# GATB/MindTheGap

Hardware: AMD Instinct MI355X
Metric: breakpoints filled/sec (higher is better)
Workload: dtype u64; 1 GPU; synthetic human-scale: 3 Gbp i.i.d. donor as 600000 x 5 kb sequences, 100000 insertion sites (50-1000 nt) per batch, k=31, max-nodes 100; sites_per_batch=100000, sites_per_rank_and_step=100000, distinct_batches_per_rank=4, site_set=400000, donor_sequences=600000, erroneous_fragments=0, k=31, max_nodes=100, max_length=10000, nb_solid_kmers=3108581096, nb_unitigs=600024, index_bytes=60154587216, unitig_store_bytes=3945966160, batches_in_flight=6, input=prepared batches, resident in HBM, output=C-ABI records + ASCII sequences in page-locked host memory

## Files before the change

### mindthegap_amd/csrc/mtg_gpu_fill.hip

```cpp
#include "mtg_gpu_common.h"

namespace mtgi {

enum { TRAVERSAL_SETS = mtg_index::NWS };
__constant__ Index c_ix[TRAVERSAL_SETS];
__constant__ FillCfg c_cfg[TRAVERSAL_SETS];

#ifndef MTG_STAGE_A_WAVES
#define MTG_STAGE_A_WAVES 2
#endif
#ifndef MTG_WALK_WAVES
#define MTG_WALK_WAVES 2
#endif
enum { PARK_LISTS = 19 };
struct ParkCtl {
    uint32_t count[PARK_LISTS];
    uint32_t n_branching;
    uint32_t pad_[3];
#ifdef MTG_BUBBLE_TIMING
    uint32_t hist_lane[32], hist_wave[32], hist_walk_lane[32], hist_walk_wave[32];
#endif
};
#ifdef MTG_BUBBLE_TIMING
__device__ __forceinline__ void timing_note(uint32_t* hl, uint32_t* hw, uint64_t t0)
// ... 950 lines not shown
            const uint32_t general_hint = ws.post_general == ~0u ? m : (uint32_t)std::min<uint64_t>(m, 4ull * ws.post_general + 1024ull);
            hipLaunchKernelGGL(k_post, dim3(general_hint), dim3(64), 0, stream, idx->dev, cfg, d_raw.as<uint8_t>(), d_head.as<uint8_t>(), d_out.as<GapOut>(), ids, d_tle, d_tbad, d_toff, d_tcnt, d_mis, d_fok,
                               in.want_all_contigs ? 1u : 0u, d_rec.as<SlotRec>(), m, park, (const uint32_t*)d_pi_head, (const uint32_t*)d_pi_next, pi_mask, d_rw, d_roff, d_tie_p);
            hipLaunchKernelGGL(k_post_lean, dim3((m + 64 / POST_LEAN_G - 1) / (64 / POST_LEAN_G)), dim3(64), 0, stream, idx->dev, cfg, d_raw.as<uint8_t>(), d_head.as<uint8_t>(), d_out.as<GapOut>(), in.want_all_contigs ? 1u : 0u, d_rec.as<SlotRec>(), m);
            const ScanBegin sbegin{{0, 0, arena_used[0], arena_used[1]}};
            hipLaunchKernelGGL(k_scan1, dim3(nblocks), dim3(SCAN_SL), 0, stream, d_rec.as<SlotRec>(), m, d_blocks.as<ScanBlock>());
            hipLaunchKernelGGL(k_scan2, dim3(1), dim3(256), 0, stream, d_blocks.as<ScanBlock>(), nblocks, sbegin, d_tot.as<PartTot>(), h_tot, park);
            HIP_TRY(hipGetLastError());
            EmitDev D;
            EmitHost H;
            const double share = std::min(1.0, std::max(0.0, tune::f(tune::T_PACKED_SEQ_SHARE, 0.0)));
            const uint32_t pack_q = (uint32_t)std::lround(share * 65536.0);
            bool packed = want_records && combo && identity && arena_used[0] == 0 && pack_q != 0;
            uint64_t shadow_halves = 0;
            if (packed) {
                shadow_halves = 2 * ((((uint64_t)sink.seq_cap * pack_q) >> 16) / 32 + 3);
                HIP_TRY(d_shadow.alloc(shadow_halves * 4));
            }
            auto emit = [&]() -> int {
                D.seq = sink.seq_dev ? sink.seq_dev : p_seq(); D.ext = d_ext.as<char>();
                D.seq_cap = sink.seq_cap; D.ext_cap = sink.ext_cap;
                D.res = p_res(); D.fil = p_fil();
                D.dense_words = d_dw.as<uint64_t>(); D.dense_meta = d_dm.as<uint32_t>();
                D.dense_cap_words = ws.cap[d_dw.slot] / 8; D.dense_cap_contigs = ws.cap[d_dm.slot] / 20;
                const bool want_wire = sink.wire_dev != nullptr && identity && tier == 0;
                D.wire = want_wire ? (uint8_t*)sink.wire_dev : nullptr; D.wire_cap = sink.wire_cap; D.wire_tag = sink.wire_tag;
                D.tot = d_tot.as<PartTot>(); D.wire_gaps = m;
                D.shadow = packed ? d_shadow.as<uint32_t>() : nullptr; D.shadow_cap = shadow_halves; D.pack_q = pack_q;
                if (packed) HIP_TRY(hipMemsetAsync(d_shadow.p, 0, shadow_halves * 4, stream));
                if (want_wire) HIP_TRY(hipMemsetAsync(sink.wire_dev, 0, sizeof(mtg_wire_header), stream));
                H.seq = sink.seq; H.ext = sink.ext; H.fil = sink.fil;
                if (!want_wire)
                    hipLaunchKernelGGL(k_emit_lean, dim3((m + 64 / EMIT_LEAN_G - 1) / (64 / EMIT_LEAN_G)), dim3(64), 0, stream, idx->dev.us, cfg, d_raw.as<uint8_t>(), d_head.as<uint8_t>(), d_rec.as<SlotRec>(), d_blocks.as<ScanBlock>(),
                                       ids, d_flags, k, D, H, m);
                hipLaunchKernelGGL(k_emit, dim3(want_wire ? m : general_hint), dim3(64), 0, stream, idx->dev.us, cfg, d_raw.as<uint8_t>(), d_head.as<uint8_t>(), d_rec.as<SlotRec>(), d_blocks.as<ScanBlock>(), ids, d_flags, k, D, H,
                                   d_rlist.as<uint32_t>(), d_glist.as<uint32_t>(), m, park, want_wire ? 0u : 1u);
                if (want_wire) hipLaunchKernelGGL(k_wire_sum, dim3(256 * 4), dim3(256), 0, stream, (uint8_t*)sink.wire_dev, sink.wire_cap);
                HIP_TRY(hipGetLastError());
                return MTG_OK;
            };
            HIP_TRY(mark(eve));
            if (int erc = emit()) return erc;
            HIP_TRY(hipEventRecord(ev2, stream));
            tick("host prep+launch");
            if (while_busy && !busy_done) { busy_done = true; (*while_busy)(); tick("host work during kernels"); }
            HIP_TRY(hipEventSynchronize(ev2));
            traversal_lock.unlock();
            tick("totals ready");
            t0 = now_ms();
            PartTot tot = *h_tot;
            const uint64_t need_w = tot.end[0] * 8 + 64, need_m = tot.end[1] * 20 + 64;
            bool again = false;
            if (want_records && tot.end[2] > sink.seq_cap) {
                const uintptr_t old = (uintptr_t)sink.seq, old_end = old + sink.seq_cap;
                const uintptr_t old_fil = (uintptr_t)sink.fil, old_fil_end = old_fil + n * sizeof(mtg_filled);
                if (!sink.grow_seq || !sink.grow_seq((size_t)tot.end[2], (size_t)tot.begin[2])) { set_error("sequence buffer too small: %llu bytes needed", (unsigned long long)tot.end[2]); return MTG_ERR_ARG; }
                if (launches > 1 && (uintptr_t)sink.seq != old)
                    for (size_t i = 0; i < n; i++) { const uintptr_t q = (uintptr_t)sink.fil[i].seq; if (q >= old && q < old_end) sink.fil[i].seq = sink.seq + (q - old); }
                if (launches > 1 && (uintptr_t)sink.fil != old_fil)
                    for (size_t i = 0; i < n; i++) { const uintptr_t q = (uintptr_t)sink.res[i].filled; if (q >= old_fil && q < old_fil_end) sink.res[i].filled = (const mtg_filled*)((const char*)sink.fil + (q - old_fil)); }
                again = true;
            }
            if (want_records && tot.end[3] > sink.ext_cap) {
                const uintptr_t old = (uintptr_t)sink.ext, old_end = old + sink.ext_cap;
                if (!sink.grow_ext || !sink.grow_ext((size_t)tot.end[3], (size_t)tot.begin[3])) { set_error("extension buffer too small: %llu bytes needed", (unsigned long long)tot.end[3]); return MTG_ERR_NOMEM; }
                if (launches > 1 && (uintptr_t)sink.ext != old)
                    for (size_t i = 0; i < n; i++) { const uintptr_t q = (uintptr_t)sink.res[i].extension; if (q >= old && q < old_end) sink.res[i].extension = sink.ext + (q - old); }
                again = true;
            }
            if (need_w > ws.cap[d_dw.slot] || need_m > ws.cap[d_dm.slot]) again = true;
            if (again) {
                HIP_TRY(hipStreamSynchronize(stream));
                if (combo) HIP_TRY(d_combo.grow_keeping(sink.combo_off_seq + std::max<size_t>(sink.seq_cap, 64) + SEQ_SLACK, sink.combo_off_seq + (size_t)tot.begin[2]));
                else if (!sink.seq_dev) HIP_TRY(d_seq.grow_keeping(std::max<size_t>(sink.seq_cap, 64) + SEQ_SLACK, (size_t)tot.begin[2]));
                HIP_TRY(d_ext.alloc(std::max<size_t>(sink.ext_cap, 64)));
                HIP_TRY(d_dw.alloc(need_w));
                HIP_TRY(d_dm.alloc(need_m));
                hipLaunchKernelGGL(k_scan1, dim3(nblocks), dim3(SCAN_SL), 0, stream, d_rec.as<SlotRec>(), m, d_blocks.as<ScanBlock>());
                hipLaunchKernelGGL(k_scan2, dim3(1), dim3(256), 0, stream, d_blocks.as<ScanBlock>(), nblocks, sbegin, d_tot.as<PartTot>(), (PartTot*)nullptr, park);
                packed = false;
                if (int erc = emit()) return erc;
            }
            CopyTurn copy_turn(idx->device);
            std::vector<mtg_gap_result> tmp_res;
            std::vector<mtg_filled> tmp_fil;
            const bool one_copy = combo && identity && tot.begin[2] == 0;
            const uint64_t pack_x = packed ? packed_split(tot.end[2], pack_q) : 0, pack_words = packed ? (tot.end[2] - pack_x + 31) / 32 : 0;
            uint64_t* h_shadow = nullptr;
            if (packed) {
                h_shadow = (uint64_t*)staging_host(&ws, Workspace::NHOST - 3, pack_words * 8 + 64);
                if (!h_shadow) { set_error("no page-locked memory for the packed sequences of a launch"); return MTG_ERR_NOMEM; }
            }
            if (want_records) {
                if (h_shadow) {
                    HIP_TRY(hipMemcpyAsync(sink.combo, d_combo.p, sink.combo_off_seq, hipMemcpyDeviceToHost, stream));
                    if (pack_words) HIP_TRY(hipMemcpyAsync(h_shadow, d_shadow.p, pack_words * 8, hipMemcpyDeviceToHost, stream));
                    HIP_TRY(hipEventRecord(evp, stream));
                    if (pack_x) HIP_TRY(hipMemcpyAsync(sink.combo + sink.combo_off_seq, (const char*)d_combo.p + sink.combo_off_seq, pack_x, hipMemcpyDeviceToHost, stream));
                } else if (one_copy) HIP_TRY(hipMemcpyAsync(sink.combo, d_combo.p, sink.combo_off_seq + (size_t)tot.end[2], hipMemcpyDeviceToHost, stream));
                else if (identity) {
                    HIP_TRY(hipMemcpyAsync(sink.res, p_res(), (size_t)m * sizeof(mtg_gap_result), hipMemcpyDeviceToHost, stream));
                    HIP_TRY(hipMemcpyAsync(sink.fil, p_fil(), (size_t)m * sizeof(mtg_filled), hipMemcpyDeviceToHost, stream));
                } else {
                    tmp_res.resize(m);
                    tmp_fil.resize(m);
                    HIP_TRY(hipMemcpyAsync(tmp_res.data(), p_res(), (size_t)m * sizeof(mtg_gap_result), hipMemcpyDeviceToHost, stream));
                    HIP_TRY(hipMemcpyAsync(tmp_fil.data(), p_fil(), (size_t)m * sizeof(mtg_filled), hipMemcpyDeviceToHost, stream));
                }
                const WireLayout wl = wire_layout(m, tot.n_filled, tot.end[2], tot.end[3]);
                const bool wired = sink.wire_dev != nullptr && identity && tier == 0 && wl.total <= sink.wire_cap && tot.n_retry == 0 && tot.n_general == 0;
                if (sink.wire_dev && identity && tier == 0) { sink.wire_ok = wired; sink.wire_bytes = wired ? wl.total : 0; }
                const char* seq_src = wired ? (const char*)sink.wire_dev + wl.o_seq : (sink.seq_dev ? sink.seq_dev : p_seq());
                if (!one_copy && !sink.seq_on_device && !sink.seq_stays_in_workspace && tot.end[2] > tot.begin[2]) HIP_TRY(hipMemcpyAsync(sink.seq + tot.begin[2], seq_src + tot.begin[2], tot.end[2] - tot.begin[2], hipMemcpyDeviceToHost, stream));
                if (tot.end[3] > tot.begin[3]) HIP_TRY(hipMemcpyAsync(sink.ext + tot.begin[3], d_ext.as<char>() + tot.begin[3], tot.end[3] - tot.begin[3], hipMemcpyDeviceToHost, stream));
            }
            std::vector<uint32_t> rlist(tot.n_retry), glist(tot.n_general);
            const bool dev_general = tot.n_general > 0 && !host_paths && !in.want_all_contigs && !tune::on(tune::T_HOST_GENERAL) && !tl_host_general;
            GenCtl* h_gctl = nullptr;
            GenDev GD{};
            if (dev_general) {
                const uint64_t ng = tot.n_general;
                HIP_TRY(d_paths.alloc(ng * (size_t)PATHS_WORDS * 4));
                HIP_TRY(d_ggaps.alloc(ng * sizeof(GenGap) + sizeof(GenCtl)));
                GD.cap_sols = 4 * ng + 1024; GD.cap_ascii = ng * 1280 + (1u << 20); GD.cap_tmp = ng * 48 + (1u << 17); GD.cap_bnd = 1u << 22;
                HIP_TRY(d_gsols.alloc(GD.cap_sols * sizeof(GenSol)));
                HIP_TRY(d_gascii.alloc(GD.cap_ascii + 64));
                HIP_TRY(d_gtmp.alloc(GD.cap_tmp * 8));
                HIP_TRY(d_gbnd.alloc(GD.cap_bnd * sizeof(NwCell)));
                GD.ctl = (GenCtl*)d_ggaps.p;
                GD.gaps = (GenGap*)((char*)d_ggaps.p + sizeof(GenCtl));
                GD.sols = d_gsols.as<GenSol>(); GD.ascii = d_gascii.as<char>(); GD.tmp = d_gtmp.as<uint64_t>(); GD.bnd = d_gbnd.as<NwCell>();
                HIP_TRY(hipMemsetAsync(GD.ctl, 0, sizeof(GenCtl), stream));
                hipLaunchKernelGGL(k_paths, dim3((unsigned)ng), dim3(64), 0, stream, cfg, d_raw.as<uint8_t>(), d_head.as<uint8_t>(), d_out.as<GapOut>(), d_glist.as<uint32_t>(), k, d_paths.as<uint32_t>(), (uint32_t)ng);
                hipLaunchKernelGGL(k_general, dim3((unsigned)ng), dim3(64), 0, stream, idx->dev, cfg, d_raw.as<uint8_t>(), d_head.as<uint8_t>(), d_out.as<GapOut>(), d_glist.as<uint32_t>(), ids, d_paths.as<uint32_t>(),
                                   d_tcnt, d_fok, d_src, d_flags, k, GD, (uint32_t)ng);
                HIP_TRY(hipGetLastError());
                h_gctl = (GenCtl*)staging_host(&ws, Workspace::NHOST - 2, sizeof(GenCtl) + ng * sizeof(GenGap) + 64);
                if (!h_gctl) { set_error("no page-locked memory for the multi-contig gaps of a launch"); return MTG_ERR_NOMEM; }
                HIP_TRY(hipMemcpyAsync(h_gctl, d_ggaps.p, sizeof(GenCtl) + ng * sizeof(GenGap), hipMemcpyDeviceToHost, stream));
            }
            HostChunk* hc = nullptr;
            SlotRec* h_rec = nullptr;
            uint64_t* h_w = nullptr;
            uint32_t* h_m = nullptr;
            const uint64_t tw = tot.end[0], tc = tot.end[1];
            if (tot.n_retry) HIP_TRY(hipMemcpyAsync(rlist.data(), d_rlist.p, (size_t)tot.n_retry * 4, hipMemcpyDeviceToHost, stream));
            auto contigs_to_host = [&]() -> int {
                hc->carve(m, tw, tc, h_rec, h_w, h_m);
                HIP_TRY(hipMemcpyAsync(h_rec, d_rec.p, (size_t)m * sizeof(SlotRec), hipMemcpyDeviceToHost, stream));
                if (tw) HIP_TRY(hipMemcpyAsync(h_w, d_dw.p, tw * 8, hipMemcpyDeviceToHost, stream));
                if (tc) HIP_TRY(hipMemcpyAsync(h_m, d_dm.p, tc * 20, hipMemcpyDeviceToHost, stream));
                return MTG_OK;
            };
            if (tot.n_general) {
                special.chunks.emplace_back(new HostChunk());
                hc = special.chunks.back().get();
                HIP_TRY(hipMemcpyAsync(glist.data(), d_glist.p, (size_t)tot.n_general * 4, hipMemcpyDeviceToHost, stream));
                if (!dev_general) { if (int crc = contigs_to_host()) return crc; }
            }
            HIP_TRY(hipEventRecord(ev3, stream));
            if (h_shadow) {
                HIP_TRY(hipEventSynchronize(evp));
                const double tx = now_ms();
                expand_packed_tail(h_shadow, sink.seq, pack_x, tot.end[2], sink.res, sink.fil, n, std::min(8, std::max(1, Pool::cpu_budget() / 2)));
                if (dbg) fprintf(stderr, "  [device_run] %-18s %.3f ms (%llu of %llu arena bytes from %llu words)\n", "packed tail", now_ms() - tx,
                                 (unsigned long long)(tot.end[2] - pack_x), (unsigned long long)tot.end[2], (unsigned long long)pack_words);
            }
            HIP_TRY(hipEventSynchronize(ev3));
            copy_turn.release();
            st.d2h_ms += now_ms() - t0;
            tick("results on the host");
            t0 = now_ms();
            st.index_lines += tot.lines; st.contig_nt += tot.contig_nt; st.store_runs += tot.store_runs; st.run_nt += tot.run_nt; st.post_lines += tot.post_lines;
            st.contig_words += tot.contig_words; st.coverage_kmers += tot.cov_kmers; st.dense_words += tw;
            st.copy_words += tot.copy_words; st.copy_cmds += tot.copy_cmds; st.coverage_direct_kmers += tot.cov_direct; st.n_lean_gaps += tot.n_lean;
            if (tier == 0 && identity) ws.post_general = m - (uint32_t)std::min<uint64_t>(tot.n_lean, m);
            st.copy_words_executed += tot.copy_words_exec; st.copy_cmds_executed += tot.copy_cmds_exec; st.post_scanned_words += tot.scan_words;
            sink.seq_used = tot.end[2];
            sink.ext_used = tot.end[3];
            arena_used[0] = tot.end[2];
            arena_used[1] = tot.end[3];
            sink.n_filled += tot.n_filled;
            if (want_records && !identity)
                for (uint32_t s2 = 0; s2 < m; s2++) { sink.res[host_ids[s2]] = tmp_res[s2]; sink.fil[host_ids[s2]] = tmp_fil[s2]; }
            for (uint32_t s2 : rlist) retry.push_back(host_ids ? host_ids[s2] : s2);
            if (tot.n_retry) sink.in_gap_order = false;
            if (hc && dev_general) {
                const uint64_t ng = tot.n_general;
                const GenCtl ctl = *h_gctl;
                const GenGap* hg = (const GenGap*)(h_gctl + 1);
                hc->gen_gaps.assign(hg, hg + ng);
                uint64_t n_host = 0;
                for (uint64_t i = 0; i < ng; i++) n_host += hg[i].status != GEN_OK;
                const uint64_t ns = std::min<uint64_t>(ctl.n_sols, GD.cap_sols), na = std::min<uint64_t>(ctl.ascii_bytes, GD.cap_ascii);
                hc->gen_sols.resize(ns);
                hc->gen_ascii.resize(na + 1);
                if (ns) HIP_TRY(hipMemcpyAsync(hc->gen_sols.data(), d_gsols.p, ns * sizeof(GenSol), hipMemcpyDeviceToHost, stream));
                if (na) HIP_TRY(hipMemcpyAsync(hc->gen_ascii.data(), d_gascii.p, na, hipMemcpyDeviceToHost, stream));
                if (host_ids) hc->gap_of.assign(host_ids, host_ids + m);
                const uint32_t chunk_id = (uint32_t)special.chunks.size() - 1;
                for (uint32_t i = 0; i < (uint32_t)ng; i++) special.special.push_back(SpecialGap{host_ids ? host_ids[glist[i]] : glist[i], chunk_id, glist[i], i});
                if (n_host) {
                    if (int crc = contigs_to_host()) return crc;
                    hc->path_of.assign(m, -1);
                    if (2 * n_host > ng) {
                        hc->paths.resize(ng * (size_t)PATHS_WORDS);
                        HIP_TRY(hipMemcpyAsync(hc->paths.data(), d_paths.p, ng * (size_t)PATHS_WORDS * 4, hipMemcpyDeviceToHost, stream));
                        for (uint32_t i = 0; i < (uint32_t)ng; i++) if (hg[i].status != GEN_OK) hc->path_of[glist[i]] = (int32_t)i;
                    } else {
                        hc->paths.resize(n_host * (size_t)PATHS_WORDS);
                        uint64_t q = 0;
                        for (uint32_t i = 0; i < (uint32_t)ng; i++)
                            if (hg[i].status != GEN_OK) {
                                HIP_TRY(hipMemcpyAsync(hc->paths.data() + q * PATHS_WORDS, d_paths.as<uint32_t>() + (size_t)i * PATHS_WORDS, (size_t)PATHS_WORDS * 4, hipMemcpyDeviceToHost, stream));
                                hc->path_of[glist[i]] = (int32_t)q++;
                            }
                    }
                }
                HIP_TRY(hipStreamSynchronize(stream));
                if (n_host) h_w[tw] = 0;
                st.n_general_host += n_host;
                st.n_general_device += ng - n_host;
            } else if (hc) {
                h_w[tw] = 0;
                if (host_ids) hc->gap_of.assign(host_ids, host_ids + m);
                const uint32_t chunk_id = (uint32_t)special.chunks.size() - 1;
                std::vector<uint32_t> pslots;
                st.n_general_host += glist.size();
                uint32_t grank = 0;
                for (uint32_t s2 : glist) {
                    special.special.push_back(SpecialGap{host_ids ? host_ids[s2] : s2, chunk_id, s2, grank++});
                    if (!host_paths && !in.want_all_contigs && h_rec[s2].p.fast == 0 && h_rec[s2].p.nb_terminal > 0) pslots.push_back(s2);
                }
                if (!pslots.empty()) {
                    HIP_TRY(d_ids.alloc(std::max<size_t>(chunk, pslots.size()) * 4));
                    HIP_TRY(hipMemcpyAsync(d_ids.p, pslots.data(), pslots.size() * 4, hipMemcpyHostToDevice, stream));
                    HIP_TRY(d_paths.alloc(pslots.size() * (size_t)PATHS_WORDS * 4));
                    hipLaunchKernelGGL(k_paths, dim3((unsigned)pslots.size()), dim3(64), 0, stream, cfg, d_raw.as<uint8_t>(), d_head.as<uint8_t>(), d_out.as<GapOut>(), d_ids.as<uint32_t>(), k,
                                       d_paths.as<uint32_t>(), (uint32_t)pslots.size());
                    HIP_TRY(hipGetLastError());
                    hc->paths.resize(pslots.size() * (size_t)PATHS_WORDS);
                    HIP_TRY(hipMemcpyAsync(hc->paths.data(), d_paths.p, hc->paths.size() * 4, hipMemcpyDeviceToHost, stream));
                    HIP_TRY(hipStreamSynchronize(stream));
                    hc->path_of.assign(m, -1);
                    for (size_t g2 = 0; g2 < pslots.size(); g2++) hc->path_of[pslots[g2]] = (int32_t)g2;
                }
            }
            st.host_ms += now_ms() - t0;
            {
// ... 106 lines not shown
```

### mindthegap_amd/csrc/mtg_host.cpp

```cpp
#include "mtg_internal.h"
#include "mtg_dict_order.h"
#include <unistd.h>

#include <algorithm>
#include <atomic>
#include <chrono>
#include <cstdio>
#include <cstdlib>
#include <cstring>
#include <mutex>
#include <set>

extern "C" {
size_t mtg_tuning_count(void) { return (size_t)mtgi::tune::T_COUNT; }
int mtg_tuning_describe(size_t i, const char** name, const char** dflt, const char** kind, const char** what)
{
    using namespace mtgi::tune;
    if (i >= (size_t)T_COUNT) { mtgi::set_error("no tuning entry %zu", i); return MTG_ERR_ARG; }
    if (name) *name = g_entries[i].name;
    if (dflt) *dflt = g_entries[i].dflt;
    if (kind) *kind = g_entries[i].kind;
    if (what) *what = g_entries[i].what;
    return MTG_OK;
}
// ... 393 lines not shown
#if defined(__x86_64__)
__attribute__((target("bmi2"))) inline uint64_t pack32_bmi2(const char* b)
{
    uint64_t c[4];
    memcpy(c, b, 32);
    const uint64_t M = 0x0606060606060606ull;
    return _pext_u64(c[0], M) | (_pext_u64(c[1], M) << 16) | (_pext_u64(c[2], M) << 32) | (_pext_u64(c[3], M) << 48);
}
const bool have_bmi2 = __builtin_cpu_supports("bmi2") && !tune::on(tune::T_NO_VEC);
#endif
inline uint64_t pack32(const char* b)
{
#if defined(__x86_64__)
    if (have_bmi2) return pack32_bmi2(b);
#endif
    uint64_t w = 0;
    for (int i = 0; i < 32; i++) w |= (uint64_t)nt_code((unsigned char)b[i]) << (2 * i);
    return w;
}
inline void pack_lsb(const char* s, size_t n, uint64_t* out)
{
    size_t i = 0, w = 0;
    for (; i + 32 <= n; i += 32) out[w++] = pack32(s + i);
    if (i < n) {
        char b[32] = {0};
        memcpy(b, s + i, n - i);
        const size_t r = n - i;
        out[w] = pack32(b) & (r < 32 ? (1ull << (2 * r)) - 1 : ~0ull);
    }
}
inline bool all_upper_acgt(const char* s, size_t n)
{
    static const struct Tab { bool ok[256]; Tab() { memset(ok, 0, sizeof ok); ok['A'] = ok['C'] = ok['G'] = ok['T'] = true; } } tab;
    bool ok = true;
    size_t i = 0;
#if defined(__x86_64__)
    static const bool vec = !tune::on(tune::T_NO_VEC);
    if (vec) {
        const __m128i A = _mm_set1_epi8('A'), C = _mm_set1_epi8('C'), G = _mm_set1_epi8('G'), T = _mm_set1_epi8('T');
        for (; i + 16 <= n; i += 16) {
            const __m128i v = _mm_loadu_si128(reinterpret_cast<const __m128i*>(s + i));
            const __m128i m = _mm_or_si128(_mm_or_si128(_mm_cmpeq_epi8(v, A), _mm_cmpeq_epi8(v, C)), _mm_or_si128(_mm_cmpeq_epi8(v, G), _mm_cmpeq_epi8(v, T)));
            if (_mm_movemask_epi8(m) != 0xFFFF) return false;
        }
    }
#endif
    for (; i < n; i++) ok &= tab.ok[(unsigned char)s[i]];
    return ok;
}
}

void expand_codes_scalar(const uint64_t* w, size_t b, size_t e, char* out)
{
    static const char NT[4] = {'A', 'C', 'T', 'G'};
    for (size_t i = b; i < e; i++) out[i] = NT[(w[i >> 5] >> (2 * (i & 31))) & 3];
}
#if defined(__x86_64__)
__attribute__((target("avx2"))) static void expand_codes_avx2(const uint64_t* w, size_t b, size_t e, char* out)
{
    size_t i = b;
    const size_t head = std::min(e, (b + 31) & ~(size_t)31);
    expand_codes_scalar(w, i, head, out);
    i = head;
    const __m256i spread = _mm256_setr_epi8(0, 0, 0, 0, 1, 1, 1, 1, 2, 2, 2, 2, 3, 3, 3, 3, 4, 4, 4, 4, 5, 5, 5, 5, 6, 6, 6, 6, 7, 7, 7, 7);
    const __m256i field = _mm256_set1_epi32((int)0xC0300C03u), low = _mm256_set1_epi8(0x0F);
    const __m256i lut = _mm256_setr_epi8('A', 'C', 'T', 'G', 'C', 0, 0, 0, 'T', 0, 0, 0, 'G', 0, 0, 0, 'A', 'C', 'T', 'G', 'C', 0, 0, 0, 'T', 0, 0, 0, 'G', 0, 0, 0);
    for (; i + 32 <= e; i += 32) {
        __m256i t = _mm256_and_si256(_mm256_shuffle_epi8(_mm256_set1_epi64x((long long)w[i >> 5]), spread), field);
        t = _mm256_and_si256(_mm256_or_si256(t, _mm256_srli_epi16(t, 4)), low);
        _mm256_storeu_si256(reinterpret_cast<__m256i*>(out + i), _mm256_shuffle_epi8(lut, t));
    }
    expand_codes_scalar(w, i, e, out);
}
static const bool have_avx2 = __builtin_cpu_supports("avx2") && !tune::on(tune::T_NO_VEC);
#endif
void expand_codes(const uint64_t* w, size_t b, size_t e, char* out)
{
#if defined(__x86_64__)
    if (have_avx2) { expand_codes_avx2(w, b, e, out); return; }
#endif
    expand_codes_scalar(w, b, e, out);
}

void expand_packed_tail(const uint64_t* w, char* seq, uint64_t x, uint64_t end, const mtg_gap_result* res, const mtg_filled* fil, size_t n, int nthreads)
{
    if (end <= x || n == 0) return;
    const size_t pieces = std::min<size_t>(n, 256);
    auto first_fill = [&](size_t g, size_t lim) { while (g < lim && res[g].n_filled == 0) g++; return g; };
    auto start_of = [&](size_t g) { return (uint64_t)(fil[g].seq - seq); };
    parallel_for(pieces, nthreads, [&](size_t c) {
        const size_t g0 = n * c / pieces, g1 = n * (c + 1) / pieces;
        const size_t f = first_fill(g0, g1);
        if (f == g1) return;
        const size_t nf = first_fill(g1, n);
        const uint64_t lo = std::max<uint64_t>(start_of(f), x), hi = std::min<uint64_t>(nf < n ? start_of(nf) : end, end);
        if (hi <= lo) return;
        expand_codes(w, lo - x, hi - x, seq + x);
        for (size_t g = f + 1; g < g1; g++) {
            if (res[g].n_filled == 0) continue;
            const uint64_t z = start_of(g) - 1;
            if (z >= lo && z < hi) seq[z] = 0;
        }
        seq[hi - 1] = 0;
    }, 1);
}

void FillInput::set_common(size_t g, std::string_view source, std::string_view swf_target, int nb_mis, uint8_t gap_flags)
{
    flags[g] = gap_flags;
    const uint64_t kfields = kmask(k);
    char sb[32] = {0};
    memcpy(sb, source.data(), (size_t)k);
    const uint64_t sp = pack32(sb) & kfields;
    src[g] = reverse_fields(sp) >> (64 - 2 * k);
    const size_t rl = swf_target.size(), w0 = roff[g];
    const size_t nw = (rl + 31) / 32 + 1;
    rwords[w0 + nw - 1] = 0;
    if (nw >= 2) rwords[w0 + nw - 2] = 0;
    pack_lsb(swf_target.data(), rl, rwords.p + w0);
    r0[g] = rl >= (size_t)k ? reverse_fields(rwords[w0] & kfields) >> (64 - 2 * k) : 0;
    if (!all_upper_acgt(swf_target.data(), rl)) { rlen[g] = 0xFFFFFFFFu; r0[g] = 0; }
    nbmis[g] = (uint8_t)nb_mis;
    bool ok = (int)source.size() == k;
    if (ok) {
        uint64_t c[4];
        memcpy(c, sb, 32);
        ok = ((c[0] | c[1] | c[2] | c[3]) & 0x0808080808080808ull) == 0;
    }
    fast_ok[g] = ok ? 1 : 0;
}
void FillInput::set_target(size_t o, std::string_view seq)
{
    uint8_t* slot = traw.p + o * TARGET_SLOT;
    const bool usable = (int)seq.size() >= k;
    memset(slot, 0, TARGET_SLOT);
    if (usable) memcpy(slot, seq.data(), (size_t)k);
    slot[TARGET_SLOT - 1] = usable ? 1 : 0;
}
struct ContigGraph {
    std::vector<std::vector<int>> in_edges;
    ContigGraph(const GapDev& gc, int k)
    {
        const uint32_t n = gc.o.n_contigs;
        in_edges.resize(n);
        const uint64_t mk1 = kmask(k - 1);
        auto kmer_at = [&](uint32_t c, uint32_t start) {
            const uint64_t* w = gc.words + gc.word_start[c];
            uint64_t f = 0;
            for (int j = 0; j < k - 1; j++) { uint32_t i = start + j; f = (f << 2) | ((w[i >> 5] >> (2 * (i & 31))) & 3ull); }
            return f & mk1;
        };
        std::unordered_map<uint64_t, std::vector<int>> by_prefix;
        for (uint32_t j = 0; j < n; j++) by_prefix[kmer_at(j, 0)].push_back((int)j);
        for (uint32_t i = 0; i < n; i++) {
            auto it = by_prefix.find(kmer_at(i, gc.len[i] - (k - 1)));
            if (it == by_prefix.end()) continue;
            for (int j : it->second) {
                if (j == (int)i && (int)gc.len[i] == k - 1) continue;
                in_edges[j].push_back((int)i);
            }
        }
        for (auto& v : in_edges) { std::sort(v.begin(), v.end()); v.erase(std::unique(v.begin(), v.end()), v.end()); }
    }
};

typedef std::vector<int> Path;
typedef std::set<std::pair<Path, int>> PathSet;

struct RevDfs {
    const ContigGraph& g;
    const std::vector<TermInfo>& terms;
    int terminal_node, target;
    int nb_calls = 0;
    bool success = true;
    static const size_t max_breadth = 20;
    std::set<Path> run(int start_node, const Path& current)
    {
        std::set<Path> paths;
        if (nb_calls++ > 10000000) { success = false; return paths; }
        if (start_node != terminal_node)
            for (auto& t : terms) if (t.node == start_node) return paths;
        if (start_node == 0) { paths.insert(current); return paths; }
        for (int next : g.in_edges[start_node]) {
            if (std::find(current.begin(), current.end(), next) == current.end()) {
                Path ext;
                ext.reserve(current.size() + 1);
                ext.push_back(next);
// ... 1497 lines not shown
```

### mindthegap_amd/csrc/mtg_internal.h

```cpp
#ifndef MTG_INTERNAL_H
#define MTG_INTERNAL_H
#include "../../include/mtg_fill.h"
#include "mtg_hostutil.h"
#include "mtg_paths.h"
#include "mtg_general.h"
#include "mtg_emit.h"
#include "mtg_copy.h"
#include "mtg_format.h"
#include "mtg_tuning.h"
#include <algorithm>
#include <atomic>
#include <condition_variable>
#include <cstdio>
#include <cstdlib>
#include <cstring>
#include <functional>
#include <memory>
#include <mutex>
#include <sched.h>
#include <string>
#include <string_view>
#include <thread>
#include <vector>

namespace mtgi {
struct Workspace {
    enum { NSLOTS = 40, NHOST = 16, NEVENTS = 16 };
    enum { SLOT_TEXT_BLOCK = 2, SLOT_SEQ = 14, SLOT_RES = 16, SLOT_FIL = 17, SLOT_FMT0 = 32 };
    void* ptr[NSLOTS] = {nullptr};
    size_t cap[NSLOTS] = {0};
    void* hptr[NHOST] = {nullptr};
    size_t hcap[NHOST] = {0};
    void* events[NEVENTS] = {nullptr};
    void* stream = nullptr;
    void* copy_stream = nullptr;
    uint32_t park_share = ~0u;
    uint32_t branch_share = ~0u;
    uint32_t post_general = ~0u;
    std::mutex mtx;
};
}

struct mtg_index {
    mtg::Index dev{};
#ifndef MTG_NWS
#define MTG_NWS 6
#endif
    enum { NWS = MTG_NWS };
    mutable std::atomic<uint32_t> branch_share_any{~0u};
    mutable std::atomic<uint32_t> park_share_any{0};
    mutable mtgi::Workspace ws[NWS];
    int device = 0;
    mtg_index_info info{};
    std::vector<mtg_build_phase> build_phases;
    uint64_t build_peak_bytes = 0;
    double build_total_ms = 0;
};

namespace mtgi {
struct WorkspaceLock {
    Workspace* ws = nullptr;
    std::unique_lock<std::mutex> lk;
};
inline WorkspaceLock acquire_workspace(const mtg_index* idx)
{
    for (int i = 0; i < mtg_index::NWS; i++) {
        std::unique_lock<std::mutex> lk(idx->ws[i].mtx, std::try_to_lock);
        if (lk.owns_lock()) return WorkspaceLock{&idx->ws[i], std::move(lk)};
    }
    static std::atomic<unsigned> turn{0};
    Workspace& w = idx->ws[turn.fetch_add(1, std::memory_order_relaxed) % mtg_index::NWS];
    return WorkspaceLock{&w, std::unique_lock<std::mutex>(w.mtx)};
}
}

namespace mtgi {

void set_error(const char* fmt, ...);

class Pool {
public:
    static Pool& get() { static Pool p; return p; }
    void run(int nworkers, const std::function<void()>& job)
    {
        std::unique_lock<std::mutex> run_lock(run_mtx_);
        const int helpers = std::min<int>(nworkers - 1, (int)threads_.size());
        if (helpers > 0) {
            {
                std::lock_guard<std::mutex> lk(m_);
                job_ = &job;
                active_.store(helpers, std::memory_order_relaxed);
                to_start_.store(helpers, std::memory_order_release);
                gen_.fetch_add(1, std::memory_order_release);
            }
            if (helpers >= (int)threads_.size()) cv_.notify_all();
            else for (int i = 0; i < helpers; i++) cv_.notify_one();
        }
        job();
        if (helpers > 0) {
            const int unclaimed = to_start_.exchange(0, std::memory_order_acq_rel);
            if (unclaimed > 0) active_.fetch_sub(unclaimed, std::memory_order_acq_rel);
            for (int spin = 0; spin < SPIN && active_.load(std::memory_order_acquire) != 0; spin++) cpu_relax();
            if (active_.load(std::memory_order_acquire) != 0) {
                std::unique_lock<std::mutex> lk(m_);
                done_cv_.wait(lk, [&] { return active_.load(std::memory_order_acquire) == 0; });
            }
            job_ = nullptr;
        }
    }
    int size() const { return (int)threads_.size() + 1; }
// ... 52 lines not shown
            bool mine = false;
            for (int spin = 0; spin < SPIN && !mine; spin++) {
                if (stop_.load(std::memory_order_relaxed)) return;
                const uint64_t g = gen_.load(std::memory_order_acquire);
                if (g != seen) { seen = g; mine = claim(); }
                else cpu_relax();
            }
            if (!mine) {
                std::unique_lock<std::mutex> lk(m_);
                cv_.wait(lk, [&] { return stop_.load() || gen_.load(std::memory_order_acquire) != seen; });
                if (stop_.load()) return;
                seen = gen_.load(std::memory_order_acquire);
                mine = claim();
            }
            if (!mine) continue;
            (*job_)();
            if (active_.fetch_sub(1, std::memory_order_acq_rel) == 1) {
                std::lock_guard<std::mutex> lk(m_);
                done_cv_.notify_all();
            }
        }
    }
    std::vector<std::thread> threads_;
    std::mutex m_, run_mtx_;
    std::condition_variable cv_, done_cv_;
    const std::function<void()>* job_ = nullptr;
    std::atomic<int> to_start_{0}, active_{0};
    std::atomic<uint64_t> gen_{0};
    std::atomic<bool> stop_{false};
};

template <typename F> inline void parallel_for(size_t n, int nthreads, F f, size_t grain = 64)
{
    if (nthreads <= 0) nthreads = Pool::get().size();
    if ((size_t)nthreads * grain > n) nthreads = (int)std::max<size_t>(n / grain, 1);
    if (nthreads <= 1) { for (size_t i = 0; i < n; i++) f(i); return; }
    std::atomic<size_t> next{0};
    std::function<void()> work = [&]() {
        for (;;) {
            const size_t b = next.fetch_add(grain);
            if (b >= n) break;
            const size_t e = std::min(n, b + grain);
            for (size_t i = b; i < e; i++) f(i);
        }
    };
    Pool::get().run(nthreads, work);
}

template <typename G> inline uint64_t parallel_prefix(size_t n, int nthreads, uint64_t* out, G get)
{
    const size_t B = 4096, nb = (n + B - 1) / B;
    std::vector<uint64_t> bs(nb + 1, 0);
    out[0] = 0;
    parallel_for(nb, nthreads, [&](size_t b) {
        uint64_t sum = 0;
        for (size_t i = b * B; i < std::min(n, (b + 1) * B); i++) { const uint64_t v = get(i); out[i + 1] = v; sum += v; }
        bs[b + 1] = sum;
    }, 1);
    for (size_t b = 0; b < nb; b++) bs[b + 1] += bs[b];
    parallel_for(nb, nthreads, [&](size_t b) {
        uint64_t run = bs[b];
        for (size_t i = b * B; i < std::min(n, (b + 1) * B); i++) { run += out[i + 1]; out[i + 1] = run; }
    }, 1);
    return bs[nb];
}

struct Target {
    std::string_view seq, name;
    bool is_rc = false;
};
struct TargetSpan {
    const Target* p = nullptr;
    uint32_t n = 0;
    size_t size() const { return n; }
    const Target& operator[](size_t i) const { return p[i]; }
    const Target* begin() const { return p; }
    const Target* end() const { return p + n; }
};

void* staging_host(Workspace* ws, int slot, size_t bytes);
void expand_codes(const uint64_t* w, size_t b, size_t e, char* out);
void expand_codes_scalar(const uint64_t* w, size_t b, size_t e, char* out);
void expand_packed_tail(const uint64_t* w, char* seq, uint64_t x, uint64_t end, const mtg_gap_result* res, const mtg_filled* fil, size_t n, int nthreads);
void* pinned_alloc(size_t bytes);
void pinned_free(void* p);
int host_register(void* p, size_t bytes);
int host_unregister(void* p);
int device_download(const mtg_index* idx, void* host_dst, const void* dev_src, size_t bytes);
int device_upload(const mtg_index* idx, void* dev_dst, const void* host_src, size_t bytes);

template <typename T> struct Arr {
    T* p = nullptr;
    size_t n = 0;
    T* data() const { return p; }
    size_t size() const { return n; }
    bool empty() const { return n == 0; }
    T& operator[](size_t i) const { return p[i]; }
};
struct FillInput {
    int k = 31;
    bool want_all_contigs = false;
    Workspace* ws = nullptr;
    Arr<uint64_t> src;
    Arr<uint64_t> r0;
    Arr<uint32_t> roff;
    Arr<uint32_t> rlen;
    Arr<uint32_t> toff, tcnt;
    Arr<uint8_t> nbmis, fast_ok, flags;
    Arr<uint64_t> rwords;
    Arr<uint8_t> traw;
    void *block_a = nullptr, *block_b = nullptr, *block_c = nullptr;
    size_t bytes_a = 0, bytes_b = 0, bytes_c = 0;
    std::vector<uint64_t> own_a, own_b, own_c;
    void* dev_a = nullptr; void* dev_b = nullptr; void* dev_tenc = nullptr;
    bool text_mode = false;
    uint64_t n_rwords = 0, n_text_targets = 0, text_bytes = 0;
    const char* text_direct = nullptr;
    struct Shared {
        const uint64_t* enc = nullptr;
        uint32_t n = 0;
        const uint32_t* pi = nullptr;
        uint32_t pi_mask = 0;
    } shared;
    uint8_t* tie_out = nullptr;
    static size_t text_block_off(size_t n, size_t nt, int which)
    {
        const size_t o[6] = {0, 8 * n, 16 * n, 16 * n + 8 * nt, 20 * n + 8 * nt, (20 * n + 12 * nt + 7) & ~(size_t)7};
        return o[which];
    }
    void resize(size_t n);
    void size(size_t i, size_t swf_len, size_t n_targets) { rlen[i] = (uint32_t)swf_len; tcnt[i] = (uint32_t)n_targets; }
    void layout();
    void set_common(size_t i, std::string_view source, std::string_view swf_target, int nb_mis, uint8_t gap_flags);
    void set_target(size_t slot, std::string_view seq);
    enum { BLOCK = 512 };
    std::vector<uint64_t> blk_rw, blk_nt;
    std::vector<uint32_t> slen;
    void alloc_b(uint64_t rw, uint64_t nt);
    template <typename SizeFn> void plan(size_t n, int nthreads, SizeFn sz)
    {
        resize(n);
        slen.resize(n);
        const size_t nb = (n + BLOCK - 1) / BLOCK;
        blk_rw.assign(nb + 1, 0);
        blk_nt.assign(nb + 1, 0);
        parallel_for(nb, nthreads, [&](size_t b) {
            uint64_t rw = 0, nt = 0;
            for (size_t i = b * BLOCK; i < std::min(n, (b + 1) * (size_t)BLOCK); i++) {
                size_t sl = 0, tn = 0;
                sz(i, sl, tn);
                size(i, sl, tn);
                rw += (sl + 31) / 32 + 1;
                nt += tn;
            }
            blk_rw[b + 1] = rw;
            blk_nt[b + 1] = nt;
        }, 1);
        for (size_t b = 0; b < nb; b++) { blk_rw[b + 1] += blk_rw[b]; blk_nt[b + 1] += blk_nt[b]; }
        alloc_b(blk_rw[nb], blk_nt[nb]);
    }
    template <typename SizeFn, typename SetFn> bool plan_and_fill(size_t n, int nthreads, SizeFn sz, SetFn st)
    {
        resize(n);
        slen.resize(n);
        const size_t nb = (n + BLOCK - 1) / BLOCK;
        blk_rw.assign(nb + 1, 0);
// ... 262 lines not shown
```

### mindthegap_amd/csrc/mtg_tuning.h

```cpp
#ifndef MTG_TUNING_H
#define MTG_TUNING_H
#include <stddef.h>
#include <stdio.h>
#include <stdlib.h>
#include <string.h>
#include <mutex>
#include <string>

#define MTG_TUNABLES(X) \
    X(POOL_THREADS, "", "cap", "size of the host worker pool (default: the CPUs the process may use -- hardware threads, affinity mask, cgroup quota -- at most 64); read when the pool starts") \
    X(PACKED_SEQ_SHARE, "0.75", "cap", "share (0..1) of a whole-batch launch's sequence arena that crosses the link 2-bit packed, the host expanding it to ASCII (0: every byte as ASCII)") \
    X(COPY_SLOTS, "3", "cap", "batches of a device that copy their results to the host at the same time (0: no limit); more copies at once share the link worse") \
    X(UPLOAD_OWN_STREAM, "", "ab", "every batch uploads its input on its own stream instead of the device's one upload stream (three uploads at a time take the link from the downloads: profiles/r04_text_entry.txt)") \
    X(SPARSE_ADJ_LOAD, "0.49", "cap", "load factor of the sparse junction table, as a share of the dense one's; 0.7 overflows the displacement range at human scale") \
    X(JT_LOAD, "0.7", "cap", "load factor of the lean build's junction table") \
    X(BLOOM_BITS, "12", "cap", "Bloom filter bits per k-mer (0: no filter, no sequence scan)") \
    X(LOAD_THREADS, "", "cap", "threads that stream a container's abundance bytes to the device (default: up to 8)") \
    X(LOAD_PIECE, "", "test", "k-mers per piece when an index container is loaded (default 2^26): small pieces exercise the piece loop") \
    X(COUNT_PASSES, "", "test", "force this many passes of the k-mer counting (default: as many as HBM needs)") \
    X(ROUNDS, "", "ab", "bubble rounds between launches of the walk kernel (default: 6 when most gaps of the previous launch parked, else 0)") \
    X(LIGHT_WALK, "", "ab", "1 / 0: the first walk of a launch by the light kernel (simple paths only, every branching node parks) / by the full one; default: light when fewer than 1 in 128 gaps of the previous launch met a branching node") \
    X(BUILD_PARTITIONED, "", "ab", "the junction table of packed sequences built partition by partition in LDS (1) or by scattered insertion (0); default: partitioned from 2^27 junction positions on") \
    X(NO_SPLIT_LONG, "", "test", "index construction from packed sequences: a sequence of more than 131 072 nucleotides stays one work item (no pieces of 65 536 that share k - 1 nucleotides)") \
    X(BUILD_POSITIONAL, "", "ab", "packed sequences: the chains that lie whole in one sequence are found by position (1, default) or every chain is walked on the junction table (0)") \
    X(FINISH_G, "", "ab", "lanes per parked gap in the finishing kernel: 1, 8, 16 or 64 (default: 64 while few gaps park, 16 otherwise)") \
    X(FINISH_WAVE_BELOW, "2048", "ab", "a whole wave per parked gap while the previous launch parked fewer gaps than this") \
    X(NO_POST_INDEX, "", "test", "the terminal search counts every contig position against every target of its gap (no piece index of the batch's dictionaries)") \
    X(NO_LEAN, "", "test", "every contig is materialised (no lean gaps)") \
    X(NO_DEFER, "", "test", "the lanes of the traversal copy their long runs themselves (no copy commands, no k_copy work)") \
    X(MAX_CHUNK, "", "test", "gaps per traversal launch (default: what the scratch holds): several launches per batch") \
    X(HOST_GENERAL, "", "test", "the multi-contig gaps by the host's path (candidate sequences, de-duplication, coverage: as until round 4) instead of k_general") \
    X(HOST_PATHS, "", "test", "leave the path enumeration of multi-contig gaps to the host") \
    X(DEBUG_SKIP_FINISH, "", "diag", "parked gaps stay parked (and fail as overflowing gaps)") \
    X(KERNEL_TIMERS, "", "diag", "every batch records an event between its kernels and mtg_last_batch_stats carries each kernel's own time (off: three events per batch instead of nine, only device_span_ms)") \
    X(DEBUG_TIMERS, "", "diag", "per-phase wall times of every batch and every index construction on stderr") \
    X(NO_VEC, "", "test", "scalar instead of vector host code (pext in the input pass, AVX2 in the expansion of a packed arena)") \
    X(NO_PREFETCH, "", "test", "no software prefetch in the input pass") \
    X(NB_GPUS, "", "cap", "the tool: devices to use (default: all visible; -nb-gpus overrides)") \
    X(CLI_BATCH, "", "cap", "the tool: sites per batch (default 100 000)") \
    X(CLI_IN_FLIGHT, "", "cap", "the tool: worker threads per device (default 3, at most 6)") \
    X(CLI_WRITERS, "1", "cap", "the tool: writer threads per output file (a file's lock serialises write(2): more than one per file was measured the same or slower)") \
    X(CLI_NO_MMAP, "", "test", "the tool reads its breakpoint file instead of mapping it") \
    X(CONTIG_PER_SEED, "", "ab", "contig mode (the tool and mtg_fill_seeds): every seed gets its own copy of the dictionary (mtg_fill_batch, as until round 6) instead of the shared table on the device") \
    X(HOST_FORMAT, "", "ab", "the tool: every site's text by the host's writers (round 3) instead of the device's formatter") \
    X(TOOL_TIMERS, "", "diag", "the tool: where the time of a run went (stderr)") \
    X(TOOL_QUIET, "", "diag", "the tool: no summary on stdout")

namespace mtgi {
namespace tune {
enum Id {
#define MTG_TUNE_ENUM(name, dflt, kind, what) T_##name,
    MTG_TUNABLES(MTG_TUNE_ENUM)
#undef MTG_TUNE_ENUM
    T_COUNT
};
struct Entry { const char* name; const char* env; const char* dflt; const char* kind; const char* what; };
inline const Entry g_entries[T_COUNT] = {
#define MTG_TUNE_ROW(name, dflt, kind, what) {#name, "MTG_" #name, dflt, kind, what},
    MTG_TUNABLES(MTG_TUNE_ROW)
#undef MTG_TUNE_ROW
};
struct Values {
    std::mutex m;
    char v[T_COUNT][64];
    bool forced[T_COUNT];
    Values()
    {
        memset(v, 0, sizeof v);
        memset(forced, 0, sizeof forced);
        if (const char* e = getenv("MTG_TUNING")) {
            std::string all(e);
            size_t b = 0;
            while (b < all.size()) {
                size_t c = all.find(',', b);
                if (c == std::string::npos) c = all.size();
                const std::string item = all.substr(b, c - b);
                const size_t eq = item.find('=');
                const std::string nm = item.substr(0, eq), val = eq == std::string::npos ? "1" : item.substr(eq + 1);
                const int t = find(nm.c_str());
                if (t >= 0) put(t, val.c_str());
                else fprintf(stderr, "MTG_TUNING: no entry named %s (mtg_tuning_describe lists them)\n", nm.c_str());
                b = c + 1;
            }
        }
    }
    static int find(const char* name)
    {
        if (!name) return -1;
        if (!strncmp(name, "MTG_", 4)) name += 4;
        for (int t = 0; t < T_COUNT; t++) if (!strcmp(g_entries[t].name, name)) return t;
        return -1;
    }
    bool put(int t, const char* val)
    {
// ... 30 lines not shown
```

Before: 228.0 million breakpoints/s.

## Overlap packed-tail host expansion with chunked D2H copies using helper threads

The packed 2-bit sequence tail is now copied device-to-host in up to 16 chunks, each followed by an event. The batch thread expands pieces whose data has already arrived while later chunks are still crossing the link. A persistent helper-thread pool picks up released pieces, and the copy turn is released as soon as the copies finish rather than after the expansion. An optional non-temporal AVX2 store path is added but is off by default; the cost is more events, thread coordination and polling overhead.

```diff
diff --git a/mindthegap_amd/csrc/mtg_gpu_fill.hip b/mindthegap_amd/csrc/mtg_gpu_fill.hip
--- a/mindthegap_amd/csrc/mtg_gpu_fill.hip
+++ b/mindthegap_amd/csrc/mtg_gpu_fill.hip
@@ -1056,6 +1056,10 @@
                 if (int erc = emit()) return erc;
             }
             CopyTurn copy_turn(idx->device);
+            const double t_turn = now_ms();
+            std::vector<hipEvent_t> tail_ev;
+            std::vector<uint64_t> tail_end;
+            enum : uint64_t { MAX_TAIL_CHUNKS = 16 };
             std::vector<mtg_gap_result> tmp_res;
             std::vector<mtg_filled> tmp_fil;
             const bool one_copy = combo && identity && tot.begin[2] == 0;
@@ -1068,8 +1072,18 @@
             if (want_records) {
                 if (h_shadow) {
                     HIP_TRY(hipMemcpyAsync(sink.combo, d_combo.p, sink.combo_off_seq, hipMemcpyDeviceToHost, stream));
-                    if (pack_words) HIP_TRY(hipMemcpyAsync(h_shadow, d_shadow.p, pack_words * 8, hipMemcpyDeviceToHost, stream));
                     HIP_TRY(hipEventRecord(evp, stream));
+                    uint64_t cw = (uint64_t)std::max(1l, tune::i(tune::T_PACKED_SEQ_CHUNK, 2l << 20) / 8);
+                    if ((pack_words + cw - 1) / cw > MAX_TAIL_CHUNKS) cw = (pack_words + MAX_TAIL_CHUNKS - 1) / MAX_TAIL_CHUNKS;
+                    for (uint64_t o = 0; o < pack_words; o += cw) {
+                        const uint64_t e = std::min(pack_words, o + cw);
+                        HIP_TRY(hipMemcpyAsync(h_shadow + o, (const uint64_t*)d_shadow.p + o, (e - o) * 8, hipMemcpyDeviceToHost, stream));
+                        hipEvent_t evk;
+                        HIP_TRY(events.make(evk));
+                        HIP_TRY(hipEventRecord(evk, stream));
+                        tail_ev.push_back(evk);
+                        tail_end.push_back(e);
+                    }
                     if (pack_x) HIP_TRY(hipMemcpyAsync(sink.combo + sink.combo_off_seq, (const char*)d_combo.p + sink.combo_off_seq, pack_x, hipMemcpyDeviceToHost, stream));
                 } else if (one_copy) HIP_TRY(hipMemcpyAsync(sink.combo, d_combo.p, sink.combo_off_seq + (size_t)tot.end[2], hipMemcpyDeviceToHost, stream));
                 else if (identity) {
@@ -1136,9 +1150,41 @@
             if (h_shadow) {
                 HIP_TRY(hipEventSynchronize(evp));
                 const double tx = now_ms();
-                expand_packed_tail(h_shadow, sink.seq, pack_x, tot.end[2], sink.res, sink.fil, n, std::min(8, std::max(1, Pool::cpu_budget() / 2)));
-                if (dbg) fprintf(stderr, "  [device_run] %-18s %.3f ms (%llu of %llu arena bytes from %llu words)\n", "packed tail", now_ms() - tx,
-                                 (unsigned long long)(tot.end[2] - pack_x), (unsigned long long)tot.end[2], (unsigned long long)pack_words);
+                TailExpansion tail(h_shadow, sink.seq, pack_x, tot.end[2], sink.res, sink.fil, n, &TailHelpers::get(), tune::on(tune::T_EXPAND_STREAM));
+                size_t ci = 0;
+                bool polled = false;
+                double t_copied = 0;
+                auto advance = [&](bool block) -> hipError_t {
+                    while (ci < tail_ev.size()) {
+                        const hipError_t e = block ? hipEventSynchronize(tail_ev[ci]) : hipEventQuery(tail_ev[ci]);
+                        if (e == hipErrorNotReady) { polled = true; return hipSuccess; }
+                        if (e != hipSuccess) return e;
+                        tail.arrived(tail_end[ci++]);
+                        block = false;
+                    }
+                    if (copy_turn.held) {
+                        const hipError_t e = hipEventQuery(ev3);
+                        if (e == hipErrorNotReady) { polled = true; return hipSuccess; }
+                        if (e != hipSuccess) return e;
+                        copy_turn.release();
+                        t_copied = now_ms();
+                    }
+                    return hipSuccess;
+                };
+                for (unsigned own = 0;;) {
+                    if ((own & 3) == 0) HIP_TRY(advance(false));
+                    if (tail.step()) { own++; continue; }
+                    if (ci == tail_ev.size()) break;
+                    HIP_TRY(advance(true));
+                    own = 0;
+                }
+                if (polled) (void)hipGetLastError();
+                HIP_TRY(hipEventSynchronize(ev3));
+                if (copy_turn.held) { copy_turn.release(); t_copied = now_ms(); }
+                tail.finish();
+                if (dbg) fprintf(stderr, "  [device_run] %-18s %.3f ms (%llu of %llu arena bytes from %llu words in %zu chunks; turn held %.3f ms, %.3f ms of expansion after the last copy; %zu of %zu pieces on the batch's thread)\n",
+                                 "packed tail", now_ms() - tx, (unsigned long long)(tot.end[2] - pack_x), (unsigned long long)tot.end[2], (unsigned long long)pack_words, tail_ev.size(),
+                                 t_copied - t_turn, now_ms() - t_copied, tail.own_pieces(), tail.pieces());
             }
             HIP_TRY(hipEventSynchronize(ev3));
             copy_turn.release();
diff --git a/mindthegap_amd/csrc/mtg_host.cpp b/mindthegap_amd/csrc/mtg_host.cpp
--- a/mindthegap_amd/csrc/mtg_host.cpp
+++ b/mindthegap_amd/csrc/mtg_host.cpp
@@ -499,27 +499,151 @@
     expand_codes_scalar(w, b, e, out);
 }
 
+#if defined(__x86_64__)
+__attribute__((target("avx2"))) static void expand_codes_avx2_stream(const uint64_t* w, size_t b, size_t e, char* out)
+{
+    size_t i = b;
+    const size_t head = std::min(e, (b + 31) & ~(size_t)31);
+    expand_codes_scalar(w, i, head, out);
+    i = head;
+    const __m256i spread = _mm256_setr_epi8(0, 0, 0, 0, 1, 1, 1, 1, 2, 2, 2, 2, 3, 3, 3, 3, 4, 4, 4, 4, 5, 5, 5, 5, 6, 6, 6, 6, 7, 7, 7, 7);
+    const __m256i field = _mm256_set1_epi32((int)0xC0300C03u), low = _mm256_set1_epi8(0x0F);
+    const __m256i lut = _mm256_setr_epi8('A', 'C', 'T', 'G', 'C', 0, 0, 0, 'T', 0, 0, 0, 'G', 0, 0, 0, 'A', 'C', 'T', 'G', 'C', 0, 0, 0, 'T', 0, 0, 0, 'G', 0, 0, 0);
+    for (; i + 32 <= e; i += 32) {
+        __m256i t = _mm256_and_si256(_mm256_shuffle_epi8(_mm256_set1_epi64x((long long)w[i >> 5]), spread), field);
+        t = _mm256_and_si256(_mm256_or_si256(t, _mm256_srli_epi16(t, 4)), low);
+        _mm256_stream_si256(reinterpret_cast<__m256i*>(out + i), _mm256_shuffle_epi8(lut, t));
+    }
+    _mm_sfence();
+    expand_codes_scalar(w, i, e, out);
+}
+#endif
+void expand_codes_stream(const uint64_t* w, size_t b, size_t e, char* out)
+{
+#if defined(__x86_64__)
+    if (have_avx2 && ((uintptr_t)out & 31) == 0) { expand_codes_avx2_stream(w, b, e, out); return; }
+#endif
+    expand_codes(w, b, e, out);
+}
+
+TailHelpers::TailHelpers(int nthreads)
+{
+    for (int i = 0; i < nthreads; i++) threads_.emplace_back([this] { loop(); });
+}
+TailHelpers::~TailHelpers()
+{
+    { std::lock_guard<std::mutex> lk(m_); stop_ = true; }
+    cv_.notify_all();
+    for (auto& t : threads_) t.join();
+}
+TailHelpers& TailHelpers::get()
+{
+    static TailHelpers h(tune::is_set(tune::T_EXPAND_HELPERS) ? (int)std::max(0l, std::min(tune::i(tune::T_EXPAND_HELPERS), 64l)) : std::min(8, Pool::get().size() / 2));
+    return h;
+}
+void TailHelpers::offer(TailExpansion* t, size_t released)
+{
+    if (threads_.empty() || released == 0) return;
+    int wake;
+    {
+        std::lock_guard<std::mutex> lk(m_);
+        if (!t->offered_) { t->offered_ = true; tasks_.push_back(t); }
+        wake = (int)std::min<size_t>(released, (size_t)sleeping_);
+    }
+    for (int i = 0; i < wake; i++) cv_.notify_one();
+}
+void TailHelpers::withdraw(TailExpansion* t)
+{
+    std::unique_lock<std::mutex> lk(m_);
+    if (!t->offered_) return;
+    tasks_.erase(std::find(tasks_.begin(), tasks_.end(), t));
+    t->offered_ = false;
+    left_cv_.wait(lk, [&] { return t->inside_ == 0; });
+}
+void TailHelpers::loop()
+{
+    std::unique_lock<std::mutex> lk(m_);
+    for (;;) {
+        TailExpansion* t = nullptr;
+        for (size_t i = 0; i < tasks_.size() && !t; i++) {
+            TailExpansion* c = tasks_[(turn_ + i) % tasks_.size()];
+            if (c->next_.load(std::memory_order_relaxed) < c->ready_.load(std::memory_order_acquire)) { t = c; turn_ = (turn_ + i + 1) % tasks_.size(); }
+        }
+        if (!t) {
+            if (stop_) return;
+            sleeping_++;
+            cv_.wait(lk);
+            sleeping_--;
+            continue;
+        }
+        t->inside_++;
+        lk.unlock();
+        while (t->take()) {}
+        lk.lock();
+        if (--t->inside_ == 0) left_cv_.notify_all();
+    }
+}
+
+TailExpansion::TailExpansion(const uint64_t* w, char* seq, uint64_t x, uint64_t end, const mtg_gap_result* res, const mtg_filled* fil, size_t n, TailHelpers* helpers,
+                             bool stream, size_t max_pieces)
+    : w_(w), seq_(seq), x_(x), end_(end), res_(res), fil_(fil), n_(n), helpers_(helpers), stream_(stream)
+{
+    if (end <= x || n == 0) return;
+    words_ = (end - x + 31) / 32;
+    npieces_ = std::max<size_t>(1, std::min<size_t>(n, max_pieces));
+    bound_.assign(npieces_ + 1, end);
+    for (size_t c = npieces_; c-- > 0;) {
+        size_t g = n * c / npieces_;
+        const size_t g1 = n * (c + 1) / npieces_;
+        while (g < g1 && res[g].n_filled == 0) g++;
+        bound_[c] = g < g1 ? std::min<uint64_t>(std::max<uint64_t>((uint64_t)(fil[g].seq - seq), x), end) : bound_[c + 1];
+    }
+}
+void TailExpansion::arrived(uint64_t words)
+{
+    size_t r = released_;
+    while (r < npieces_ && (bound_[r + 1] - x_ + 31) / 32 <= words) r++;
+    if (r == released_) return;
+    const size_t more = r - released_;
+    released_ = r;
+    ready_.store(r, std::memory_order_release);
+    if (helpers_ && more > 1) helpers_->offer(this, more - 1);
+}
+bool TailExpansion::take()
+{
+    size_t c = next_.load(std::memory_order_relaxed);
+    do {
+        if (c >= ready_.load(std::memory_order_acquire)) return false;
+    } while (!next_.compare_exchange_weak(c, c + 1, std::memory_order_acq_rel, std::memory_order_relaxed));
+    run_piece(c);
+    return true;
+}
+void TailExpansion::run_piece(size_t c)
+{
+    const uint64_t lo = bound_[c], hi = bound_[c + 1];
+    if (hi <= lo) return;
+    if (stream_) expand_codes_stream(w_, lo - x_, hi - x_, seq_ + x_);
+    else expand_codes(w_, lo - x_, hi - x_, seq_ + x_);
+    for (size_t g = n_ * c / npieces_, g1 = n_ * (c + 1) / npieces_; g < g1; g++) {
+        if (res_[g].n_filled == 0) continue;
+        const uint64_t z = (uint64_t)(fil_[g].seq - seq_) - 1;
+        if (z >= lo && z < hi) seq_[z] = 0;
+    }
+    seq_[hi - 1] = 0;
+}
+void TailExpansion::finish()
+{
+    if (finished_) return;
+    finished_ = true;
+    arrived(words_);
+    while (step()) {}
+    if (helpers_) helpers_->withdraw(this);
+}
+
 void expand_packed_tail(const uint64_t* w, char* seq, uint64_t x, uint64_t end, const mtg_gap_result* res, const mtg_filled* fil, size_t n, int nthreads)
 {
-    if (end <= x || n == 0) return;
-    const size_t pieces = std::min<size_t>(n, 256);
-    auto first_fill = [&](size_t g, size_t lim) { while (g < lim && res[g].n_filled == 0) g++; return g; };
-    auto start_of = [&](size_t g) { return (uint64_t)(fil[g].seq - seq); };
-    parallel_for(pieces, nthreads, [&](size_t c) {
-        const size_t g0 = n * c / pieces, g1 = n * (c + 1) / pieces;
-        const size_t f = first_fill(g0, g1);
-        if (f == g1) return;
-        const size_t nf = first_fill(g1, n);
-        const uint64_t lo = std::max<uint64_t>(start_of(f), x), hi = std::min<uint64_t>(nf < n ? start_of(nf) : end, end);
-        if (hi <= lo) return;
-        expand_codes(w, lo - x, hi - x, seq + x);
-        for (size_t g = f + 1; g < g1; g++) {
-            if (res[g].n_filled == 0) continue;
-            const uint64_t z = start_of(g) - 1;
-            if (z >= lo && z < hi) seq[z] = 0;
-        }
-        seq[hi - 1] = 0;
-    }, 1);
+    TailExpansion t(w, seq, x, end, res, fil, n, nthreads > 1 ? &TailHelpers::get() : nullptr);
+    t.finish();
 }
 
 void FillInput::set_common(size_t g, std::string_view source, std::string_view swf_target, int nb_mis, uint8_t gap_flags)
diff --git a/mindthegap_amd/csrc/mtg_internal.h b/mindthegap_amd/csrc/mtg_internal.h
--- a/mindthegap_amd/csrc/mtg_internal.h
+++ b/mindthegap_amd/csrc/mtg_internal.h
@@ -25,7 +25,7 @@
 
 namespace mtgi {
 struct Workspace {
-    enum { NSLOTS = 40, NHOST = 16, NEVENTS = 16 };
+    enum { NSLOTS = 40, NHOST = 16, NEVENTS = 32 };
     enum { SLOT_TEXT_BLOCK = 2, SLOT_SEQ = 14, SLOT_RES = 16, SLOT_FIL = 17, SLOT_FMT0 = 32 };
     void* ptr[NSLOTS] = {nullptr};
     size_t cap[NSLOTS] = {0};
@@ -244,6 +244,57 @@
 void expand_codes(const uint64_t* w, size_t b, size_t e, char* out);
 void expand_codes_scalar(const uint64_t* w, size_t b, size_t e, char* out);
 void expand_packed_tail(const uint64_t* w, char* seq, uint64_t x, uint64_t end, const mtg_gap_result* res, const mtg_filled* fil, size_t n, int nthreads);
+void expand_codes_stream(const uint64_t* w, size_t b, size_t e, char* out);
+
+class TailExpansion;
+class TailHelpers {
+public:
+    explicit TailHelpers(int nthreads);
+    ~TailHelpers();
+    static TailHelpers& get();
+    int size() const { return (int)threads_.size(); }
+    void offer(TailExpansion* t, size_t released);
+    void withdraw(TailExpansion* t);
+private:
+    void loop();
+    std::vector<std::thread> threads_;
+    std::mutex m_;
+    std::condition_variable cv_, left_cv_;
+    std::vector<TailExpansion*> tasks_;
+    size_t turn_ = 0;
+    int sleeping_ = 0;
+    bool stop_ = false;
+};
+class TailExpansion {
+public:
+    enum { PIECES = 256 };
+    TailExpansion(const uint64_t* w, char* seq, uint64_t x, uint64_t end, const mtg_gap_result* res, const mtg_filled* fil, size_t n, TailHelpers* helpers,
+                  bool stream = false, size_t max_pieces = PIECES);
+    ~TailExpansion() { if (helpers_) helpers_->withdraw(this); }
+    TailExpansion(const TailExpansion&) = delete;
+    TailExpansion& operator=(const TailExpansion&) = delete;
+    uint64_t words() const { return words_; }
+    void arrived(uint64_t words);
+    bool step() { if (!take()) return false; own_++; return true; }
+    void finish();
+    size_t pieces() const { return npieces_; }
+    size_t own_pieces() const { return own_; }
+private:
+    friend class TailHelpers;
+    bool take();
+    void run_piece(size_t c);
+    const uint64_t* w_;
+    char* seq_;
+    uint64_t x_, end_, words_ = 0;
+    const mtg_gap_result* res_;
+    const mtg_filled* fil_;
+    size_t n_, npieces_ = 0, released_ = 0, own_ = 0;
+    std::vector<uint64_t> bound_;
+    TailHelpers* helpers_;
+    bool stream_, offered_ = false, finished_ = false;
+    std::atomic<size_t> next_{0}, ready_{0};
+    int inside_ = 0;
+};
 void* pinned_alloc(size_t bytes);
 void pinned_free(void* p);
 int host_register(void* p, size_t bytes);
diff --git a/mindthegap_amd/csrc/mtg_tuning.h b/mindthegap_amd/csrc/mtg_tuning.h
--- a/mindthegap_amd/csrc/mtg_tuning.h
+++ b/mindthegap_amd/csrc/mtg_tuning.h
@@ -10,6 +10,9 @@
 #define MTG_TUNABLES(X) \
     X(POOL_THREADS, "", "cap", "size of the host worker pool (default: the CPUs the process may use -- hardware threads, affinity mask, cgroup quota -- at most 64); read when the pool starts") \
     X(PACKED_SEQ_SHARE, "0.75", "cap", "share (0..1) of a whole-batch launch's sequence arena that crosses the link 2-bit packed, the host expanding it to ASCII (0: every byte as ASCII)") \
+    X(PACKED_SEQ_CHUNK, "2097152", "cap", "bytes of the packed tail per copy: the tail crosses the link in pieces of this size (at most 16 per batch) and the host expands what has arrived while the rest is on the link") \
+    X(EXPAND_HELPERS, "", "cap", "threads that help the batches' own threads expand packed tails (default: half the worker pool's size, at most 8; 0: every batch expands alone); read when the first packed tail arrives") \
+    X(EXPAND_STREAM, "", "ab", "the expansion of a packed tail writes with non-temporal stores (profiles/packed_pieces_ab.txt: faster in two runs of three at share 1, not decided)") \
     X(COPY_SLOTS, "3", "cap", "batches of a device that copy their results to the host at the same time (0: no limit); more copies at once share the link worse") \
     X(UPLOAD_OWN_STREAM, "", "ab", "every batch uploads its input on its own stream instead of the device's one upload stream (three uploads at a time take the link from the downloads: profiles/r04_text_entry.txt)") \
     X(SPARSE_ADJ_LOAD, "0.49", "cap", "load factor of the sparse junction table, as a share of the dense one's; 0.7 overflows the displacement range at human scale") \
```

New measurement: 216.6 million breakpoints/s. 5.0% lower.
